# yashnaray/VQ-VAE-HMM-model

Measured on AMD Instinct MI355X. Metric: VAE_HMM train-step sequences/sec (K=3, T=200, D=5) at 1/2/4/8 MI355X, higher is better.
Workload: dtype f32; 1 GPU; cfg2: VAE_HMM train step (compute_loss+backward+Adam); global_batch=1024, per_gpu_batch=1024, seq_len=200, K=3, input_dim=5, hidden_dim=64, hidden_dim2=32, u_dim=4, trans_hidden=128, parallelism=single, hip_graph=False, step_form=fused (Adam in the backward's tail launch), eager

## Files before the change

### vq-vae-hmm-model_amd/csrc/strip.hip

```cpp
#include "vqhmm.h"

#include <stddef.h>
#include <stdlib.h>

#include "prof.h"
#include "strip_dev.h"

namespace vqhmm {

struct StripFwdArgs {
  int64_t R;
  int T, D, H2, K, P;
  const float* xp;
  const float *img_e1, *img_d1;
  const float *img_e2, *img_d2;
  const float *b_e1, *b_e2, *b_d1, *b_d2;
  const float *tWl, *tbl;
  const float *tWp, *tbp;
  float *h1e, *h2e, *logits, *q, *g1, *g2, *par;
  int64_t nstrip;
  int dbg;
};

namespace {

template <int NB2>
struct StripFwdLds {
  static constexpr int NW2 = 16 * NB2;
  float We2[3 * NW2 * ST_LDW];
  float Wd2[3 * 64 * ST_LDW];
  float Ee2[NW2 * 17 + 16];
  float Ed2[64 * 17 + 16];
  float Wf[2][3 * 64 * 8];
  float bf[2][64];
  float Xx[ST_XR * ST_XLD];
  float Xq[ST_XR * ST_XLD];
  float slot[8][18 * ST_LDW];
  unsigned long long hcnt[8];
};

template <int TH>
struct StripHeadW {
  static constexpr int LDW2 = TH + 4;
  float W2S[16 * LDW2];
  float W1S[TH * 8];
};
struct StripHeadLds {
  static constexpr int LDL = 20;
  float uS[ST_WIN * 8];
  float lgS[ST_WIN * LDL];
  float dlgS[ST_WIN * LDL];
  float aS[ST_WIN * 4];
  float wS[ST_WIN];
  double red[8][4];
  float q0w[8][4];
};

__device__ __forceinline__ void pk_weights(const float* Wf, int C, int lg4, int l16, float (&w)[4][4]) {
#pragma unroll
  for (int e = 0; e < 4; ++e) {
    const int k = 4 * lg4 + e;
    const bool in = k < 3 * C;
    const int tap = in ? k / C : 0, c = in ? k - tap * C : 0;
#pragma unroll
    for (int nb = 0; nb < 4; ++nb) {
      const float v = Wf[(tap * 64 + nb * 16 + l16) * 8 + c];
      w[nb][e] = in ? v : 0.f;
    }
  }
}

__device__ __forceinline__ void pk_block(const float (&w)[4][4], const float* Xw, int C, int lg4, int l16,
                                         f32x4 (&acc)[4]) {
  float b[4];
#pragma unroll
  for (int e = 0; e < 4; ++e) {
    const int k = 4 * lg4 + e;
    const bool in = k < 3 * C;
    const int tap = in ? k / C : 0, c = in ? k - tap * C : 0;
    const float v = Xw[(l16 + tap) * ST_XLD + c];
    b[e] = in ? v : 0.f;
  }
#pragma unroll
  for (int nb = 0; nb < 4; ++nb) {
    acc[nb] = f32x4{0.f, 0.f, 0.f, 0.f};
#pragma unroll
    for (int e = 0; e < 4; ++e) acc[nb] = mfma16x16x4(w[nb][e], b[e], acc[nb]);
  }
}

__device__ __forceinline__ void front_epi(f32x4 (&acc)[4], const f32x4 (&bias)[4], int64_t r0, int64_t R, int T,
                                          int lg4, int l16, int slo, int shi, float* out, float* xs,
                                          bool nostore, int only = -1, float* xlo = nullptr,
                                          float* xhi = nullptr) {
  const int64_t r = r0 + l16;
  const bool valid = row_valid(r, R, T);
  const bool st = l16 >= slo && l16 < shi && r < R && !nostore;
#pragma unroll
  for (int nb = 0; nb < 4; ++nb) {
    f32x4 y;
#pragma unroll
    for (int v = 0; v < 4; ++v) {
      const float yy = relu_f(acc[nb][v] * 1.0f + bias[nb][v]);
      y[v] = valid ? yy : 0.f;
    }
    acc[nb] = y;
    if (st) *reinterpret_cast<f32x4*>(out + r * 64 + nb * 16 + 4 * lg4) = y;
    if (only < 0 || l16 == only) *reinterpret_cast<f32x4*>(xs + l16 * ST_LDW + nb * 16 + 4 * lg4) = y;
    if (xlo && l16 == 0) *reinterpret_cast<f32x4*>(xlo + nb * 16 + 4 * lg4) = y;
    if (xhi && l16 == 15) *reinterpret_cast<f32x4*>(xhi + nb * 16 + 4 * lg4) = y;
  }
}

template <int NB>
struct TailConsts {
  f32x4 bias[NB], tw[NB], tb;
  __device__ __forceinline__ void load(const float* Es, int lg4, int l16) {
    constexpr int NW = 16 * NB;
#pragma unroll
    for (int nb = 0; nb < NB; ++nb) {
      const float4 b4 = *reinterpret_cast<const float4*>(Es + nb * 16 + 4 * lg4);
      const float4 t4 = *reinterpret_cast<const float4*>(Es + NW + l16 * NW + nb * 16 + 4 * lg4);
      bias[nb] = f32x4{b4.x, b4.y, b4.z, b4.w};
      tw[nb] = f32x4{t4.x, t4.y, t4.z, t4.w};
    }
    const float4 t4 = *reinterpret_cast<const float4*>(Es + 17 * NW + 4 * lg4);
    tb = f32x4{t4.x, t4.y, t4.z, t4.w};
  }
};

template <int NB, bool SM>
__device__ __forceinline__ void tail_epi(f32x4 (&acc)[NB], const TailConsts<NB>& k, int64_t r0, int64_t R, int T,
                                         int lg4, int l16, int slo, int shi, int N, float* out, int C2, float* t_out,
                                         float* q_out, float* xq, bool nostore) {
  const int64_t r = r0 + l16;
  const bool valid = row_valid(r, R, T);
  const bool st = l16 >= slo && l16 < shi && r < R && !nostore;
  const int ldn = ld4(N), ldt = ld4(C2);
#pragma unroll
  for (int nb = 0; nb < NB; ++nb) {
    f32x4 y;
#pragma unroll
    for (int v = 0; v < 4; ++v) {
      const float yy = relu_f(acc[nb][v] * 1.0f + k.bias[nb][v]);
      y[v] = valid ? yy : 0.f;
    }
    acc[nb] = y;
    const int n0 = nb * 16 + 4 * lg4;
    if (st && n0 < ldn) *reinterpret_cast<f32x4*>(out + r * ldn + n0) = y;
  }
  f32x4 z = k.tb;
#pragma unroll
  for (int nb = 0; nb < NB; ++nb)
#pragma unroll
    for (int v = 0; v < 4; ++v) z = mfma16x16x4(k.tw[nb][v], acc[nb][v], z);
  const int c0 = 4 * lg4;
#pragma unroll
  for (int v = 0; v < 4; ++v) z[v] = valid ? z[v] : 0.f;
  if (st && c0 < ldt) *reinterpret_cast<f32x4*>(t_out + r * ldt + c0) = z;
  if constexpr (SM) {
    float m = -__builtin_inff();
#pragma unroll
    for (int v = 0; v < 4; ++v)
      if (c0 + v < C2) m = fmaxf(m, z[v]);
    m = fmaxf(m, xor16(m));
    m = fmaxf(m, xor32(m));
    float e[4], s = 0.f;
#pragma unroll
    for (int v = 0; v < 4; ++v) {
      e[v] = (c0 + v < C2) ? __expf(z[v] - m) : 0.f;
      s += e[v];
    }
    s += xor16(s);
    s += xor32(s);
    f32x4 qv;
#pragma unroll
    for (int v = 0; v < 4; ++v) qv[v] = valid ? e[v] / s : 0.f;
    if (st && c0 < ldt) *reinterpret_cast<f32x4*>(q_out + r * ldt + c0) = qv;
    if (c0 == 0) {
      *reinterpret_cast<f32x4*>(xq + l16 * ST_XLD) = qv;
      *reinterpret_cast<f32x4*>(xq + l16 * ST_XLD + 4) = z;
    }
  }
}

template <int NW>
__device__ __forceinline__ const float* es_src(const float* bias, int N, const float* tW, const float* tb, int C2, int i,
                                               bool& ok) {
  const bool in_b = i < NW, in_w = !in_b && i < 17 * NW;
  const int j = in_w ? i - NW : 0, c2w = j / NW, n = j - c2w * NW, c2b = (!in_b && !in_w) ? i - 17 * NW : 0;
  ok = in_b ? i < N : in_w ? (c2w < C2 && n < N) : c2b < C2;
// ... 12 lines not shown
}
__device__ __forceinline__ float row4_max(float v) {
  v = fmaxf(v, dppf<0xB1>(v));
  v = fmaxf(v, dppf<0x4E>(v));
  return v;
}
__device__ __forceinline__ float row4_reduce_scatter(const float (&c)[4], int i) {
  const bool hi2 = i & 2, hi1 = i & 1;
  float h2[2];
#pragma unroll
  for (int k = 0; k < 2; ++k) {
    const float send = hi2 ? c[k] : c[2 + k];
    h2[k] = (hi2 ? c[2 + k] : c[k]) + dppf<0x4E>(send);
  }
  const float send = hi1 ? h2[0] : h2[1];
  return (hi1 ? h2[1] : h2[0]) + dppf<0xB1>(send);
}
}

template <int NB2, int PROF, int HTH>
__global__ __launch_bounds__(512) void strip_fwd_kernel(StripFwdArgs a, HeadArgs h) {
  using S = StripFwdLds<NB2>;
  constexpr int NW2 = S::NW2;
  extern __shared__ float4 smem4[];
  S& sh = *reinterpret_cast<S*>(smem4);
  const int tid = threadIdx.x, lane = tid & 63, wave = tid >> 6;
  const int lg4 = lane >> 4, l16 = lane & 15;
  const int64_t R = a.R;
  const int T = a.T, ldx = ld4(a.D);
  float* slot = sh.slot[wave];

  auto load_x = [&](int64_t s0) {
    const int row = tid >> 1, h = 4 * (tid & 1);
    int64_t r = s0 - 2 + row;
    r = r < 0 ? 0 : (r >= R ? R - 1 : r);
    return *reinterpret_cast<const float4*>(a.xp + r * ldx + (h < ldx ? h : 0));
  };
  auto store_x = [&](int64_t s0, float4 v) {
    if (tid < 2 * ST_XR) {
      const int row = tid >> 1, h = 4 * (tid & 1);
      const int64_t r = s0 - 2 + row;
      const bool ok = r >= 0 && r < R && h < ldx;
      *reinterpret_cast<float4*>(sh.Xx + row * ST_XLD + h) = ok ? v : make_float4(0.f, 0.f, 0.f, 0.f);
    }
  };

  constexpr int HKP = 4, HB = HTH > 0 ? HTH / 16 : 1, HLDW2 = HTH + 4, HNW = HTH > 0 ? 16 * HLDW2 + HTH * 8 : 1;
  constexpr int HNJ = (HNW + 511) / 512;
  const int prow = tid >> 2, si = tid & 3;
  float hwv[HNJ];
  if constexpr (HTH > 0) {
    const int KK = h.K * h.K;
#pragma unroll
    for (int j = 0; j < HNJ; ++j) {
      const int i = tid + 512 * j;
      float v = 0.f;
      if (i < 16 * HLDW2) {
        const int ij = i / HLDW2, hh = i - ij * HLDW2;
        v = (ij < KK && hh < HTH) ? h.W2[ij * HTH + hh] : 0.f;
      } else if (i < HNW) {
        const int k = i - 16 * HLDW2, hh = k >> 3, c = k & 7;
        v = c < h.U ? h.W1[hh * h.U + c] : (c == h.U ? h.b1[hh] : 0.f);
      }
      hwv[j] = v;
    }
    if (!h.norm && !h.cnt_in) {
      unsigned long long c = 0;
      for (int64_t b = tid; b < h.B; b += 512) {
        const int64_t L = h.lengths[b];
        c += (unsigned long long)(L <= 0 ? 0 : (L < T ? L : T));
      }
#pragma unroll
      for (int o = 32; o >= 1; o >>= 1) c += __shfl_xor(c, o);
      if (lane == 0) sh.hcnt[wave] = c;
    }
  }
  stamp<PROF>(0);
  if constexpr (PROF > 0) { if (threadIdx.x == 0 && blockIdx.x < 256) g_prof[blockIdx.x * 16 + 13] = __builtin_amdgcn_s_memtime(); }
  for (int j = wave; wave < 4 && j < 12; j += 4) {
    const int g = j * 64 + lane, img = g / 384, i = g - img * 384, row = i >> 1, h = 4 * (i & 1);
    dma16((img ? a.img_d1 : a.img_e1) + row * ST_LDF + h, &sh.Wf[0][0] + j * 256);
  }
  int64_t s = blockIdx.x;
  float4 px = load_x(s * ST_OWN - ST_HALO);
  constexpr int NE = NW2 * 17 + 16, ND = 64 * 17 + 16, NC = NE + ND + 128;
  constexpr int NCJ = (NC + 511) / 512;
  float cv[NCJ];
  bool cvok[NCJ];
#pragma unroll
  for (int j = 0; j < NCJ; ++j) {
    const int i = tid + 512 * j;
    bool oke, okd;
    const float* pe = es_src<NW2>(a.b_e2, a.H2, a.tWl, a.tbl, a.K, i < NE ? i : 0, oke);
    const float* pd = es_src<64>(a.b_d2, 64, a.tWp, a.tbp, a.P, (i >= NE && i < NE + ND) ? i - NE : 0, okd);
    const int ib = (i >= NE + ND && i < NC) ? i - NE - ND : 0;
    const bool inE = i < NE, inD = !inE && i < NE + ND, inB = !inE && !inD && i < NC;
    const bool ok = inE ? oke : inD ? okd : inB;
    const float* p = inE ? pe : inD ? pd : (ib < 64 ? a.b_e1 : a.b_d1) + (ib & 63);
    cv[j] = *(ok ? p : a.b_e1);
    cvok[j] = ok;
  }
#pragma unroll
  for (int j = 0; j < NCJ; ++j) cv[j] = cvok[j] ? cv[j] : 0.f;
  {
    constexpr int N1 = 3 * NW2 * ST_LDW / 4, N2 = 3 * 64 * ST_LDW / 4;
    constexpr int C1 = (N1 + 63) / 64, C2 = (N2 + 63) / 64;
    constexpr int NJ = (C1 + C2 + 7) / 8;
#pragma unroll
    for (int jj = 0; jj < NJ; ++jj) {
      const int c = min(wave + 8 * jj, C1 + C2 - 1);
      const bool first = c < C1;
      const int cc = first ? c : c - C1;
      const int i = cc * 64 + lane;
      if (i < (first ? N1 : N2)) dma16((first ? a.img_e2 : a.img_d2) + 4 * i, (first ? sh.We2 : sh.Wd2) + cc * 256);
    }
  }
  static_assert(offsetof(S, Ed2) == offsetof(S, Ee2) + NE * 4, "constant blocks must be contiguous");
#pragma unroll
  for (int j = 0; j < NCJ; ++j) {
    const int i = tid + 512 * j;
    if (i < NE + ND) sh.Ee2[i] = cv[j];
    else if (i < NC) sh.bf[0][i - NE - ND] = cv[j];
  }
  if (tid < 4 * ST_XLD) sh.Xq[(tid < 2 * ST_XLD ? 0 : (ST_XR - 4) * ST_XLD) + tid] = 0.f;
  store_x(s * ST_OWN - ST_HALO, px);
  lds_barrier();
  stamp<PROF>(1);
  float wE[4][4], wD[4][4];
  pk_weights(sh.Wf[0], a.D, lg4, l16, wE);
  pk_weights(sh.Wf[1], a.K, lg4, l16, wD);
  f32x4 bE[4], bD[4];
#pragma unroll
  for (int nb = 0; nb < 4; ++nb) {
    const float4 e4 = *reinterpret_cast<const float4*>(sh.bf[0] + nb * 16 + 4 * lg4);
    const float4 d4 = *reinterpret_cast<const float4*>(sh.bf[1] + nb * 16 + 4 * lg4);
    bE[nb] = f32x4{e4.x, e4.y, e4.z, e4.w};
    bD[nb] = f32x4{d4.x, d4.y, d4.z, d4.w};
  }
  TailConsts<NB2> kE;
  TailConsts<4> kD;
  if constexpr (HTH == 0) {
    kE.load(sh.Ee2, lg4, l16);
    kD.load(sh.Ed2, lg4, l16);
  }
  static_assert(HTH == 0 || (offsetof(S, Xx) == offsetof(S, bf) + 2 * 64 * 4 &&
                             sizeof(StripHeadW<HTH>) <= offsetof(S, Xx) - offsetof(S, Wf) &&
                             sizeof(StripHeadLds) <= sizeof(float) * 8 * 18 * ST_LDW),
                "the head's LDS fits the regions it reuses");
  float lp_i = 0.f, inv_n = 1.f, cpri = 0.f, cent = 0.f;
  const bool hgrad = h.need_grad != 0;
  if constexpr (HTH > 0) {
    unsigned long long cnt;
    if (h.norm) cnt = (unsigned long long)h.norm[0];
    else if (h.cnt_in) cnt = (unsigned long long)*h.cnt_in;
    else cnt = ((((((sh.hcnt[0] + sh.hcnt[1]) + sh.hcnt[2]) + sh.hcnt[3]) + sh.hcnt[4]) + sh.hcnt[5]) + sh.hcnt[6]) + sh.hcnt[7];
    inv_n = 1.0f / fmaxf((float)(cnt * (unsigned long long)h.D), 1.0f);
    const float Bn = loss_norm_batch(h.norm, h.B);
    cpri = -h.beta / Bn;
    cent = h.beta / Bn;
    float m = -__builtin_inff();
    for (int k = 0; k < h.K; ++k) m = fmaxf(m, h.log_prior[k]);
    float se = 0.f;
    for (int k = 0; k < h.K; ++k) se += __expf(h.log_prior[k] - m);
    if (si < h.K) lp_i = h.log_prior[si] - (m + __logf(se));
  }
  float s_rec = 0.f, s_ent = 0.f, s_tr = 0.f, s_init = 0.f, q0acc = 0.f, db2acc = 0.f;
  f32x4 gW2 = f32x4{0.f, 0.f, 0.f, 0.f}, gW1 = gW2;

  const int mlo = ST_HALO - 16 * wave, mhi = ST_HALO + ST_OWN - 16 * wave;
  const int slo = max(0, mlo), shi = min(16, mhi);
  const bool nost = a.dbg & 1;
  int it = 0;
  for (; s < a.nstrip; s += gridDim.x) {
    const int64_t s0 = s * ST_OWN - ST_HALO;
    const int64_t rb = s0 + 16 * wave;
    {
      const int64_t nx = s + gridDim.x;
      px = load_x((nx < a.nstrip ? nx : s) * ST_OWN - ST_HALO);
    }
    {
      f32x4 acc[4];
      pk_block(wE, sh.Xx + (16 * wave + 1) * ST_XLD, a.D, lg4, l16, acc);
      front_epi(acc, bE, rb, R, T, lg4, l16, slo, shi, a.h1e, slot + ST_LDW, nost, -1,
                wave > 0 ? sh.slot[wave - 1] + 17 * ST_LDW : nullptr, wave < 7 ? sh.slot[wave + 1] : nullptr);
      if (wave == 5 || wave == 6) {
        const bool lo = wave == 5;
        f32x4 acc2[4];
        pk_block(wE, sh.Xx + (lo ? 0 : 16 * 7 + 2) * ST_XLD, a.D, lg4, l16, acc2);
        front_epi(acc2, bE, lo ? s0 - 1 : s0 + 16 * 7 + 1, R, T, lg4, l16, 0, 0, a.h1e,
                  lo ? sh.slot[0] : sh.slot[7] + 2 * ST_LDW, true, lo ? 0 : 15);
      }
    }
    if (it == 0) asm volatile("s_waitcnt vmcnt(0)" ::: "memory");
    lds_barrier();
    {
      f32x4 acc[NB2][1];
#pragma unroll
      for (int nb = 0; nb < NB2; ++nb) acc[nb][0] = f32x4{0.f, 0.f, 0.f, 0.f};
      c2_mfma_tile<NB2, 1, 4, 3, ST_LDW, NW2>(sh.We2, slot, lg4, l16, acc, true);
      f32x4 y[NB2];
#pragma unroll
      for (int nb = 0; nb < NB2; ++nb) y[nb] = acc[nb][0];
      if constexpr (HTH > 0) kE.load(sh.Ee2, lg4, l16);
      tail_epi<NB2, true>(y, kE, rb, R, T, lg4, l16, slo, shi, a.H2, a.h2e, a.K, a.logits, a.q,
                          sh.Xq + (16 * wave + 2) * ST_XLD, nost);
    }
    lds_barrier();
    if (it == 0) stamp<PROF>(2);
    if constexpr (HTH > 0) {
      if (it == 0) {
        float* hw = &sh.Wf[0][0];
#pragma unroll
        for (int j = 0; j < HNJ; ++j)
          if (tid + 512 * j < HNW) hw[tid + 512 * j] = hwv[j];
      }
    }
    {
      f32x4 acc[4];
      pk_block(wD, sh.Xq + (16 * wave + 1) * ST_XLD, a.K, lg4, l16, acc);
      if constexpr (PROF > 0) {
        if (it == 0) {
          asm volatile("s_nop 0" : : "v"(acc[3][3]));
          stamp<PROF>(10);
        }
      }
      front_epi(acc, bD, rb, R, T, lg4, l16, slo, shi, a.g1, slot + ST_LDW, nost, -1,
                wave > 0 ? sh.slot[wave - 1] + 17 * ST_LDW : nullptr, wave < 7 ? sh.slot[wave + 1] : nullptr);
      if (it == 0) stamp<PROF>(11);
    }
    lds_barrier();
    if (it == 0) stamp<PROF>(4);
    {
      f32x4 acc[4][1];
#pragma unroll
      for (int nb = 0; nb < 4; ++nb) acc[nb][0] = f32x4{0.f, 0.f, 0.f, 0.f};
      c2_mfma_tile<4, 1, 4, 3, ST_LDW, 64>(sh.Wd2, slot, lg4, l16, acc, true);
      f32x4 y[4];
#pragma unroll
      for (int nb = 0; nb < 4; ++nb) y[nb] = acc[nb][0];
      if constexpr (PROF > 0) {
        if (it == 0) {
          asm volatile("s_nop 0" : : "v"(y[3][3]));
          stamp<PROF>(5);
        }
      }
      if constexpr (HTH > 0) kD.load(sh.Ed2, lg4, l16);
      tail_epi<4, false>(y, kD, rb, R, T, lg4, l16, slo, shi, 64, a.g2, a.P, a.par, nullptr, nullptr, nost);
    }
    if (it == 0) stamp<PROF>(6);
    {
      const int64_t nx = s + gridDim.x;
      store_x((nx < a.nstrip ? nx : s) * ST_OWN - ST_HALO, px);
    }
    if constexpr (HTH > 0) __syncthreads();
    else lds_barrier();
    if (it == 0) stamp<PROF>(3);
    if constexpr (HTH > 0) {
      StripHeadLds& hs = *reinterpret_cast<StripHeadLds*>(&sh.slot[0][0]);
      const StripHeadW<HTH>& hw = *reinterpret_cast<const StripHeadW<HTH>*>(&sh.Wf[0][0]);
      constexpr int LDL = StripHeadLds::LDL;
      const int K = h.K, U = h.U, D = h.D, KK = K * K;
      const int ldp = ld4(2 * D), ldxh = ld4(D), ldu = ld4(U);
      const int64_t r = s0 + ST_HALO + prow;
      const unsigned Tp = (unsigned)T + 2u;
      const unsigned rcl = (unsigned)(r < R ? r : R - 1);
      const int b = (int)(rcl / Tp);
      const int t = (int)(rcl - (unsigned)b * Tp) - 1;
      const bool valid = r < R && prow <= ST_OWN && t >= 0 && t < T;
      const bool own = prow < ST_OWN && r < R;
      const int64_t L = h.lengths[b];
      const bool m = valid && t < L;
      const float wgt = (valid && t >= 1 && t < L) ? 1.f : 0.f;
      const float* qrow = sh.Xq + (ST_HALO + prow + 2) * ST_XLD;
      float qv[HKP];
#pragma unroll
      for (int k = 0; k < HKP; ++k) qv[k] = (valid && k < K) ? qrow[k] : 0.f;
      const float qp = (valid && t >= 1 && si < K) ? qrow[si - ST_XLD] : 0.f;
      float qi = 0.f;
#pragma unroll
      for (int k = 0; k < HKP; ++k) qi = si == k ? qv[k] : qi;
      float mu[2], lv[2], xv[2];
#pragma unroll
      for (int k = 0; k < 2; ++k) {
        const int c = min(si + HKP * k, D - 1);
        mu[k] = h.par[(int64_t)rcl * ldp + c];
        lv[k] = h.par[(int64_t)rcl * ldp + D + c];
        xv[k] = h.x[(int64_t)rcl * ldxh + c];
      }
      const float uu = h.u[(int64_t)rcl * ldu + min(si, ldu - 1)];
#pragma unroll
      for (int c = si; c < 8; c += HKP) hs.uS[prow * 8 + c] = c < U ? (valid ? uu : 0.f) : (c == U ? 1.f : 0.f);
      for (int i = tid; i < ST_WIN * LDL; i += 512)
        if (i % LDL >= KK) hs.dlgS[i] = 0.f;
      lds_barrier();
      {
        f32x4 lg;
#pragma unroll
        for (int v = 0; v < 4; ++v) {
          const int ij = 4 * lg4 + v;
          lg[v] = ij < KK ? h.b2[ij] : 0.f;
        }
        const float ub = hs.uS[(wave * 16 + l16) * 8 + lg4];
#pragma unroll 2
        for (int hb = 0; hb < HB; ++hb) {
          const float w1a = lg4 < U ? hw.W1S[(hb * 16 + l16) * 8 + lg4] : 0.f;
          f32x4 bb;
#pragma unroll
          for (int v = 0; v < 4; ++v) bb[v] = hw.W1S[(hb * 16 + 4 * lg4 + v) * 8 + U];
          const f32x4 w2v = *reinterpret_cast<const f32x4*>(&hw.W2S[l16 * HLDW2 + hb * 16 + 4 * lg4]);
          const f32x4 hc = mfma16x16x4(w1a, ub, bb);
#pragma unroll
          for (int v = 0; v < 4; ++v) lg = mfma16x16x4(w2v[v], relu_f(hc[v]), lg);
        }
        *reinterpret_cast<f32x4*>(&hs.lgS[(wave * 16 + l16) * LDL + 4 * lg4]) = lg;
      }
      lds_barrier();
      float rsj = 0.f;
      {
        float la[HKP];
        float A_i = 0.f;
        const float* lr = &hs.lgS[prow * LDL + (si < K ? si : 0) * K];
        float mx = -__builtin_inff();
#pragma unroll
        for (int j = 0; j < HKP; ++j) {
          la[j] = j < K ? lr[j] : 0.f;
          if (j < K) mx = fmaxf(mx, la[j]);
        }
        float se = 0.f;
#pragma unroll
        for (int j = 0; j < HKP; ++j)
          if (j < K) se += __expf(la[j] - mx);
        const float ls = mx + __logf(se);
#pragma unroll
        for (int j = 0; j < HKP; ++j)
          if (j < K) la[j] -= ls;
#pragma unroll
        for (int j = 0; j < HKP; ++j)
          if (j < K) A_i = fmaf(qv[j], la[j], A_i);
        if (si >= K) A_i = 0.f;
        float c[HKP];
#pragma unroll
        for (int j = 0; j < HKP; ++j) c[j] = (j < K && si < K) ? qp * la[j] : 0.f;
        rsj = row4_reduce_scatter(c, si);
        if (own && si < K) s_tr = fmaf(wgt * qp, A_i, s_tr);
        hs.aS[prow * HKP + si] = A_i;
        if (si == 0) hs.wS[prow] = wgt;
        if (hgrad && si < K) {
          float qs = 0.f;
#pragma unroll
          for (int j = 0; j < HKP; ++j)
            if (j < K) qs += qv[j];
          const float g = own ? cpri * wgt * qp : 0.f;
          const float rs = g * qs;
          float* dl = &hs.dlgS[prow * LDL + si * K];
#pragma unroll
          for (int j = 0; j < HKP; ++j)
// ... 246 lines not shown
    lds_barrier();
    f32x4 d1[4];
    {
      f32x4 acc[4][1];
#pragma unroll
      for (int nb = 0; nb < 4; ++nb) acc[nb][0] = f32x4{0.f, 0.f, 0.f, 0.f};
      c2_mfma_tile<4, 1, 4, 3, ST_LDW, 64>(sh.Wd2, slot, lg4, l16, acc, true);
#pragma unroll
      for (int nb = 0; nb < 4; ++nb) d1[nb] = acc[nb][0];
      mask_epi(d1, m1, 1.0f, rb, R, T, lg4, l16, slo, shi, a.dg1, nullptr, 0);
    }
    lds_barrier();
#pragma unroll
    for (int nb = 0; nb < 4; ++nb) *reinterpret_cast<f32x4*>(D1 + (16 * wave + 1 + l16) * ST_LDW + nb * 16 + 4 * lg4) = d1[nb];
    float4 m2[4];
    load_mask(a.h1e, rb, R, lg4, l16, m2);
    lds_barrier();
    if (it == 0) stamp<PROF>(2);
    {
      f32x4 acc1[1][1] = {{f32x4{0.f, 0.f, 0.f, 0.f}}};
      c2_mfma_tile<1, 1, 4, 3, ST_LDW, 16>(sh.Wc1, D1 + 16 * wave * ST_LDW, lg4, l16, acc1, true);
      const float zb1[1][4] = {}, tw1[1][4] = {};
      const float4 aux1[1][1] = {};
      const float fsc = f.scale ? *f.scale : 1.0f;
      conv2_epilogue<1, 1, 3>(f, rb, 0, lg4, l16, acc1, aux1, zb1, tw1, f32x4{0.f, 0.f, 0.f, 0.f}, fsc, false, slo,
                              shi, sh.Dh2 + (16 * wave + 1) * SB_LDE, SB_LDE);
    }
    lds_barrier();
    if (it == 0) stamp<PROF>(3);
    {
      f32x4 acc[4][1];
#pragma unroll
      for (int nb = 0; nb < 4; ++nb) acc[nb][0] = f32x4{0.f, 0.f, 0.f, 0.f};
      c2_mfma_tile<4, 1, 2, 3, SB_LDE, 64>(sh.We2, sh.Dh2 + 16 * wave * SB_LDE, lg4, l16, acc, true);
      f32x4 y[4];
#pragma unroll
      for (int nb = 0; nb < 4; ++nb) y[nb] = acc[nb][0];
      mask_epi(y, m2, 1.0f, rb, R, T, lg4, l16, slo, shi, a.dh1, nullptr, 0);
    }
    ++it;
  }
  if constexpr (PROF > 0) {
    __syncthreads();
    stamp<PROF>(7);
    if (threadIdx.x == 0 && blockIdx.x < 256) g_prof[blockIdx.x * 16 + 8] = (unsigned long long)it;
  }
}

bool strip_bwd_supported(const ConvArgs& pd, const ConvArgs& d2, const ConvArgs& f, const ConvArgs& e2) {
  return pd.R > 0 && pd.R < (1ll << 31) && pd.ks == 1 && pd.act == 2 && pd.Wimg && pd.aux && pd.out && pd.N == 64 &&
         pd.Kc >= 1 && pd.Kc <= 16 && !pd.src_cf && !pd.bias &&
         d2.src == pd.out && d2.ks == 3 && d2.act == 2 && d2.Wimg && d2.aux && d2.out && d2.Kc == 64 && d2.N == 64 &&
         !d2.bias && !d2.scale &&
         f.src == d2.out && f.act == 3 && f.ks == 3 && f.Wimg && f.Kc == 64 && f.N >= 1 && f.N <= 4 && f.lb_dh &&
         f.lb_C > 16 && f.lb_C <= 32 && ld4(f.lb_C) == 32 && !f.bias && !f.out_cf &&
         e2.src == f.lb_dh && e2.ks == 3 && e2.act == 2 && e2.Wimg && e2.aux && e2.out && e2.Kc == f.lb_C &&
         e2.N == 64 && !e2.bias && !e2.scale && !e2.tW && !e2.out_cf;
}

int launch_strip_bwd(const ConvArgs& pd, const ConvArgs& d2, const ConvArgs& f, const ConvArgs& e2, hipStream_t s) {
  if (!strip_bwd_supported(pd, d2, f, e2)) return VQHMM_EUNSUPPORTED;
  StripBwdArgs a{};
  a.R = pd.R; a.T = pd.T; a.ldp = ld4(pd.Kc);
  a.dpar = pd.src; a.g2 = pd.aux; a.g1 = d2.aux; a.h1e = e2.aux;
  a.img_pd = pd.Wimg; a.img_d2 = d2.Wimg; a.img_c1 = f.Wimg; a.img_e2 = e2.Wimg;
  a.gscale = pd.scale;
  a.dg2 = pd.out; a.dg1 = d2.out; a.dh1 = e2.out;
  a.nstrip = cdiv(pd.R, ST_OWN);
  const unsigned grid = (unsigned)(a.nstrip < 256 ? a.nstrip : 256);
  if (prof_on()) strip_bwd_kernel<1><<<grid, 512, sizeof(StripBwdLds), s>>>(a, f);
  else strip_bwd_kernel<0><<<grid, 512, sizeof(StripBwdLds), s>>>(a, f);
  VQHMM_LAUNCH_CHECK();
  return VQHMM_OK;
}

static StripFwdArgs strip_fwd_args(const ConvArgs& e1, const ConvArgs& e2, const ConvArgs& d1, const ConvArgs& d2) {
  StripFwdArgs a{};
  a.R = e1.R; a.T = e1.T; a.D = e1.Kc; a.H2 = e2.N; a.K = e2.C2; a.P = d2.C2;
  a.xp = e1.src;
  a.img_e1 = e1.Wimg; a.img_d1 = d1.Wimg; a.img_e2 = e2.Wimg; a.img_d2 = d2.Wimg;
  a.b_e1 = e1.bias; a.b_e2 = e2.bias; a.b_d1 = d1.bias; a.b_d2 = d2.bias;
  a.tWl = e2.tW; a.tbl = e2.tb; a.tWp = d2.tW; a.tbp = d2.tb;
  a.h1e = e1.out; a.h2e = e2.out; a.logits = e2.t_out; a.q = e2.q_out; a.g1 = d1.out; a.g2 = d2.out; a.par = d2.t_out;
  a.nstrip = cdiv(e1.R, ST_OWN);
  static const int dbg = [] {
    const char* e = VQHMM_PROF_ENV("VQHMM_STRIP_DBG");
    return e ? atoi(e) : 0;
  }();
  a.dbg = dbg;
  return a;
}

bool strip_fwd_supported(const ConvArgs& e1, const ConvArgs& e2, const ConvArgs& d1, const ConvArgs& d2) {
  auto relu3 = [](const ConvArgs& a) { return a.ks == 3 && a.act == 1 && !a.src_cf && a.Wimg && a.out && !a.out_cf; };
  return relu3(e1) && relu3(e2) && relu3(d1) && relu3(d2) && e1.R > 0 && e1.R < (1ll << 31) &&
         e1.Kc >= 1 && 3 * e1.Kc <= 16 && e1.N == 64 &&
         e2.src == e1.out && e2.Kc == 64 && e2.N >= 1 && e2.N <= 32 &&
         e2.C2 >= 1 && e2.C2 <= 4 && e2.t_out && e2.q_out && !e2.q_cf && !e2.reg_out && !e2.t_cf0 &&
         d1.src == e2.q_out && d1.Kc == e2.C2 && 3 * d1.Kc <= 16 && d1.N == 64 &&
         d2.src == d1.out && d2.Kc == 64 && d2.N == 64 && d2.C2 >= 1 && d2.C2 <= 16 && d2.t_out && !d2.t_cf0 &&
         !d2.q_out && !d2.q_cf && !d2.reg_out;
}

int strip_prof_copy(uint64_t* out, int64_t n) { return prof_copy(out, n); }

bool strip_head_supported(const HeadArgs& h) {
  return h.K >= 1 && h.K <= 4 && h.U >= 1 && h.U <= 4 && (h.TH == 64 || h.TH == 128) && h.D >= 1 && h.D <= 8 &&
         h.R < (1ll << 31);
}

int strip_fwd_grid(int64_t R) {
  const int64_t n = cdiv(R, ST_OWN);
  return (int)(n < 256 ? (n > 0 ? n : 1) : 256);
}

int launch_strip_fwd(const ConvArgs& e1, const ConvArgs& e2, const ConvArgs& d1, const ConvArgs& d2, const HeadArgs* h,
                     hipStream_t s) {
  if (!strip_fwd_supported(e1, e2, d1, d2)) return VQHMM_EUNSUPPORTED;
  if (h && (!strip_head_supported(*h) || h->K != e2.C2 || h->R != e1.R || h->D != e1.Kc)) return VQHMM_EUNSUPPORTED;
  const StripFwdArgs a = strip_fwd_args(e1, e2, d1, d2);
  const unsigned grid = (unsigned)strip_fwd_grid(e1.R);
  const HeadArgs hv = h ? *h : HeadArgs{};
  const int hth = h ? h->TH : 0;
#define VQHMM_SF(NB2, P, HT) strip_fwd_kernel<NB2, P, HT><<<grid, 512, sizeof(StripFwdLds<NB2>), s>>>(a, hv)
#define VQHMM_SF_H(NB2, P) \
  if (hth == 128) VQHMM_SF(NB2, P, 128); else if (hth == 64) VQHMM_SF(NB2, P, 64); else VQHMM_SF(NB2, P, 0);
  const bool prof = prof_on() != 0;
  if (c2_nb(e2.N) == 1) {
    if (prof) { VQHMM_SF_H(1, 1) } else { VQHMM_SF_H(1, 0) }
  } else {
    if (prof) { VQHMM_SF_H(2, 1) } else { VQHMM_SF_H(2, 0) }
  }
#undef VQHMM_SF_H
#undef VQHMM_SF
  VQHMM_LAUNCH_CHECK();
  return VQHMM_OK;
}

}
```

### vq-vae-hmm-model_amd/csrc/strip_bwdw.hip

```cpp
#include "vqhmm.h"

#include <stddef.h>

#include "prof.h"
#include "strip_dev.h"

namespace vqhmm {

__device__ float g_bwdw_one = 1.0f;

namespace {
constexpr int SW_LDD = 24;
constexpr int SW_LDQ = 8;
constexpr int SW_LO = 3;
constexpr int SW_OWN = 120;
static_assert(SW_OWN % 4 == 0 && SW_LO + SW_OWN - 1 <= ST_WIN - 4, "dh1 is exact on window rows 3 .. ST_WIN - 4");

struct StripWLds {
  float RW[3 * 64 * ST_LDW];
  float RS[8 * 18 * ST_LDW];
  float RG[ST_WIN * ST_LDW];
  float RD[(ST_WIN + 2) * SB_LDE];
  float RC[4 * 256];
  float RE[ST_WIN * SW_LDQ];
// ... 65 lines not shown
    ar[j % NS] = fa(qa, j);
#pragma unroll
    for (int t = 0; t < NT; ++t) br[j % NS][t] = fb(qb, j, t);
  };
  auto load = [&](int j) __attribute__((always_inline)) { load_at(j, pa, pb); };
  auto next = [&]() __attribute__((always_inline)) {
    pa += ga;
    pb += gb;
    hide(pa);
    hide(pb);
  };
  hide(pa);
  hide(pb);
  auto mma = [&](int j) __attribute__((always_inline)) {
    const float av = (SEL == SEL_A && !ok) ? 0.f : ar[j % NS];
    bacc += av;
#pragma unroll
    for (int t = 0; t < NT; ++t) acc[t] = mfma16x16x4(av, (SEL == SEL_B && !ok) ? 0.f : br[j % NS][t], acc[t]);
  };
  if constexpr (NT == 1) {
    if (nstep < 4) {
#pragma unroll
      for (int j = 0; j < 3; ++j)
        if (j < nstep) load(j);
#pragma unroll
      for (int j = 0; j < 3; ++j)
        if (j < nstep) mma(j);
      return;
    }
#pragma unroll
    for (int j = 0; j < 4; ++j) {
      load(j);
      asm volatile("" ::: "memory");
    }
    next();
    int k = 0;
    for (; k + 8 <= nstep; k += 4) {
#pragma unroll
      for (int j = 0; j < 4; ++j) {
        __builtin_amdgcn_sched_barrier(0);
        mma(j);
        __builtin_amdgcn_sched_barrier(0);
        load(j);
      }
      next();
    }
    const int rem = nstep - k - 4;
#pragma unroll
    for (int j = 0; j < 4; ++j) {
      __builtin_amdgcn_sched_barrier(0);
      mma(j);
      __builtin_amdgcn_sched_barrier(0);
      if (j < 3) load_at(j, j < rem ? pa : pa - ga, j < rem ? pb : pb - gb);
    }
#pragma unroll
    for (int j = 0; j < 3; ++j) {
      __builtin_amdgcn_sched_barrier(0);
      if (j < rem) mma(j);
    }
    return;
  }
  load(0);
  int k = 0;
  for (; k + 5 <= nstep; k += 4) {
#pragma unroll
    for (int j = 0; j < 4; ++j) {
      if (j == 3) next();
      load((j + 1) & 3);
      __builtin_amdgcn_sched_barrier(0);
      mma(j);
      __builtin_amdgcn_sched_barrier(0);
    }
  }
  const int rem = nstep - k;
#pragma unroll
  for (int j = 0; j < 4; ++j) {
    if (j < 3 && j + 1 < rem) load(j + 1);
    __builtin_amdgcn_sched_barrier(0);
    if (j < rem) mma(j);
    __builtin_amdgcn_sched_barrier(0);
  }
}

__device__ __forceinline__ void dma16_uncounted(const float* src, int off, float* dst) {
  const unsigned d = __builtin_amdgcn_readfirstlane((unsigned)(size_t)(__attribute__((address_space(3))) float*)dst);
  unsigned keep;
  asm volatile("s_nop 4\n\ts_mov_b32 %0, m0\n\ts_mov_b32 m0, %2\n\ts_nop 0\n\t"
               "global_load_lds_dwordx4 %1, %3\n\ts_mov_b32 m0, %0"
               : "=&s"(keep)
               : "v"(off), "s"(d), "s"(src)
               : "memory");
}

__device__ __forceinline__ float col_sum4(float v) {
  v += xor16(v);
  v += xor32(v);
  return v;
}
__device__ __forceinline__ void dec1_epi(f32x4 acc, float sc, int64_t r, int64_t R, int T, int lg4, int l16, float lsc,
                                         const f32x4 (&qdl)[3], const f32x4 (&h4)[2], const float* TWs, float* xs_dh,
                                         float* xs_dl) {
  const bool valid = row_valid(r, R, T);
  f32x4 y;
#pragma unroll
  for (int v = 0; v < 4; ++v) {
    const float yy = acc[v] * sc + 0.f;
    y[v] = valid ? yy : 0.f;
  }
  float yk[4];
#pragma unroll
  for (int k = 0; k < 4; ++k) yk[k] = __shfl(y[k], l16);
  if (r >= 0 && r < R) {
    float dq[4], sdot = 0.f;
#pragma unroll
    for (int k = 0; k < 4; ++k) {
      dq[k] = yk[k] + lsc * qdl[1][k];
      sdot = fmaf(qdl[0][k], dq[k], sdot);
    }
    float dl[4];
#pragma unroll
    for (int k = 0; k < 4; ++k) dl[k] = qdl[0][k] * (dq[k] - sdot) + lsc * qdl[2][k];
    if (lg4 == 0) *reinterpret_cast<f32x4*>(xs_dl + l16 * SW_LDQ) = f32x4{dl[0], dl[1], dl[2], dl[3]};
#pragma unroll
    for (int j = 0; j < 2; ++j) {
      const int c0 = 8 * lg4 + 4 * j;
      f32x4 o;
#pragma unroll
      for (int v = 0; v < 4; ++v) {
        float sacc = 0.f;
#pragma unroll
        for (int k = 0; k < 4; ++k) sacc = fmaf(TWs[k * 32 + c0 + v], dl[k], sacc);
        o[v] = h4[j][v] > 0.f ? sacc : 0.f;
      }
      *reinterpret_cast<f32x4*>(xs_dh + l16 * SB_LDE + c0) = o;
    }
  } else {
#pragma unroll
    for (int j = 0; j < 2; ++j) *reinterpret_cast<f32x4*>(xs_dh + l16 * SB_LDE + 8 * lg4 + 4 * j) = f32x4{0.f, 0.f, 0.f, 0.f};
    if (lg4 == 0) *reinterpret_cast<f32x4*>(xs_dl + l16 * SW_LDQ) = f32x4{0.f, 0.f, 0.f, 0.f};
  }
}
}

template <int PROF>
__global__ __launch_bounds__(512) void strip_bwdw_kernel(SWArgs a, ConvArgs f) {
  extern __shared__ float4 smem4[];
  StripWLds& sh = *reinterpret_cast<StripWLds*>(smem4);
  const int tid = threadIdx.x, lane = tid & 63, wave = tid >> 6;
  const int lg4 = lane >> 4, l16 = lane & 15;
  const int64_t R = a.R;
  const int T = a.T, own = a.own, nstep = own / 4;
  constexpr int lo = SW_LO;
  float* slot = sh.RS + wave * 18 * ST_LDW;
  if (a.step_inc && blockIdx.x == 0 && tid == 0) *a.step_inc = (*a.step_inc & 0xffffffffll) + 1;

  stamp<PROF>(0);
  if constexpr (PROF > 0) { if (tid == 0 && blockIdx.x < 256) g_prof[blockIdx.x * 16 + 13] = __builtin_amdgcn_s_memtime(); }
  const int K = a.K, D = a.D;
  float twv = 0.f;
  if (tid < 128) {
    const int k = tid >> 5, c = tid & 31;
    twv = (k < K && c < a.H2) ? f.lb_W[k * a.H2 + c] : 0.f;
  }
  {
    constexpr int NC = 3 * 4 * ST_LDW / 4;
    static_assert(NC <= 4 * 64 && sizeof(StripWLds::RC) == 4 * 1024, "one whole-chunk DMA per wave");
    const int c = min(wave, 3);
    const int i = min(c * 64 + lane, NC - 1);
    dma16(a.img_c1 + ((i / 72) * 16 * ST_LDW + (i % 72) * 4), sh.RC + c * 256);
  }
  if (tid < 128) sh.TW[tid] = twv;
  auto dma_d2 = [&]() __attribute__((always_inline)) {
    constexpr int N1 = 3 * 64 * ST_LDW / 4, C1 = N1 / 64;
    static_assert(N1 % 64 == 0 && C1 <= 56, "7 whole chunks per wave");
#pragma unroll
// ... 432 lines not shown
```

### vq-vae-hmm-model_amd/csrc/strip_dev.h

```cpp
#pragma once
#include "conv2_dev.h"

namespace vqhmm {

namespace {
constexpr int ST_WIN = 128;
constexpr int ST_HALO = 2;
constexpr int ST_OWN = ST_WIN - 2 * ST_HALO;
constexpr int ST_XR = ST_WIN + 4;
constexpr int ST_XLD = 8;
constexpr int ST_LDW = 72;
constexpr int ST_LDF = 24;
constexpr int SB_LDE = 40;

__device__ __forceinline__ bool row_valid(int64_t r, int64_t R, int T) {
  if (r < 0 || r >= R) return false;
  const unsigned Tp = (unsigned)T + 2u, m = (unsigned)r % Tp;
  return m >= 1u && m <= (unsigned)T;
}

__device__ __forceinline__ void lds_barrier_dma() { asm volatile("s_waitcnt lgkmcnt(0)\n\ts_barrier" ::: "memory"); }

__device__ __forceinline__ void dma16(const float* src, float* dst) {
  __builtin_amdgcn_global_load_lds(reinterpret_cast<const uint32_t*>(src), (__attribute__((address_space(3))) void*)dst,
                                   16, 0, 0);
}

__device__ __forceinline__ void mask_epi(f32x4 (&acc)[4], const float4 (&aux)[4], float sc, int64_t r0, int64_t R,
                                         int T, int lg4, int l16, int slo, int shi, float* out, float* xs, int xld,
                                         int only = -1, float* xlo = nullptr, float* xhi = nullptr) {
  const int64_t r = r0 + l16;
  const bool valid = row_valid(r, R, T);
  const bool st = out && l16 >= slo && l16 < shi && r < R;
#pragma unroll
  for (int nb = 0; nb < 4; ++nb) {
    const float av[4] = {aux[nb].x, aux[nb].y, aux[nb].z, aux[nb].w};
    f32x4 y;
#pragma unroll
    for (int v = 0; v < 4; ++v) {
      float yy = acc[nb][v] * sc + 0.f;
      yy = av[v] > 0.f ? yy : 0.f;
      y[v] = valid ? yy : 0.f;
    }
    acc[nb] = y;
    if (st) *reinterpret_cast<f32x4*>(out + r * 64 + nb * 16 + 4 * lg4) = y;
    if (xs && (only < 0 || l16 == only)) *reinterpret_cast<f32x4*>(xs + l16 * xld + nb * 16 + 4 * lg4) = y;
    if (xlo && l16 == 0) *reinterpret_cast<f32x4*>(xlo + nb * 16 + 4 * lg4) = y;
    if (xhi && l16 == 15) *reinterpret_cast<f32x4*>(xhi + nb * 16 + 4 * lg4) = y;
  }
}

__device__ __forceinline__ void load_mask(const float* m, int64_t r0, int64_t R, int lg4, int l16, float4 (&aux)[4]) {
  int64_t r = r0 + l16;
  r = r < 0 ? 0 : (r >= R ? R - 1 : r);
#pragma unroll
  for (int nb = 0; nb < 4; ++nb) aux[nb] = *reinterpret_cast<const float4*>(m + r * 64 + nb * 16 + 4 * lg4);
}
}

}
```

Baseline: 2.662 million sequences/s.

## Widen strip halo to drop extra edge conv blocks in strip forward

Changes the strip forward kernel's owned window from 124 rows with a 2-row halo to 122 rows starting at row 3. This lets the extra per-strip edge-row conv work done by waves 5 and 6 be removed, since the edge values are now recomputed inside the window. It also precomputes the conv gather offsets once, moves the weight-image DMA after the x store using an uncounted LDS DMA helper, and moves the next-strip x store earlier in the loop. The trade-off is slightly more strips and halo overlap, plus more reliance on hand-written asm DMA ordering.

```diff
diff --git a/vq-vae-hmm-model_amd/csrc/strip.hip b/vq-vae-hmm-model_amd/csrc/strip.hip
--- a/vq-vae-hmm-model_amd/csrc/strip.hip
+++ b/vq-vae-hmm-model_amd/csrc/strip.hip
@@ -23,6 +23,10 @@
 };
 
 namespace {
+
+constexpr int SF_LO = 3;
+constexpr int SF_OWN = 122;
+static_assert(SF_LO >= 3 && SF_LO + SF_OWN - 1 <= ST_WIN - 4, "g2 / par are exact on window rows 3 .. ST_WIN - 4");
 
 template <int NB2>
 struct StripFwdLds {
@@ -70,17 +74,30 @@
   }
 }
 
-__device__ __forceinline__ void pk_block(const float (&w)[4][4], const float* Xw, int C, int lg4, int l16,
-                                         f32x4 (&acc)[4]) {
+struct PkGather {
+  int off[4];
+  unsigned in;
+  __device__ __forceinline__ void set(int C, int lg4, int l16) {
+    in = 0;
+#pragma unroll
+    for (int e = 0; e < 4; ++e) {
+      const int k = 4 * lg4 + e;
+      const bool ok = k < 3 * C;
+      const int tap = ok ? k / C : 0, c = ok ? k - tap * C : 0;
+      off[e] = (l16 + tap) * ST_XLD + c;
+      asm volatile("" : "+v"(off[e]));
+      in |= ok ? 1u << e : 0u;
+    }
+  }
+};
+
+__device__ __forceinline__ void pk_block(const float (&w)[4][4], const float* Xw, const PkGather& g, f32x4 (&acc)[4]) {
   float b[4];
 #pragma unroll
-  for (int e = 0; e < 4; ++e) {
-    const int k = 4 * lg4 + e;
-    const bool in = k < 3 * C;
-    const int tap = in ? k / C : 0, c = in ? k - tap * C : 0;
-    const float v = Xw[(l16 + tap) * ST_XLD + c];
-    b[e] = in ? v : 0.f;
-  }
+  for (int e = 0; e < 4; ++e) b[e] = Xw[g.off[e]];
+  __builtin_amdgcn_sched_barrier(0);
+#pragma unroll
+  for (int e = 0; e < 4; ++e) b[e] = (g.in >> e & 1u) ? b[e] : 0.f;
 #pragma unroll
   for (int nb = 0; nb < 4; ++nb) {
     acc[nb] = f32x4{0.f, 0.f, 0.f, 0.f};
@@ -91,8 +108,7 @@
 
 __device__ __forceinline__ void front_epi(f32x4 (&acc)[4], const f32x4 (&bias)[4], int64_t r0, int64_t R, int T,
                                           int lg4, int l16, int slo, int shi, float* out, float* xs,
-                                          bool nostore, int only = -1, float* xlo = nullptr,
-                                          float* xhi = nullptr) {
+                                          bool nostore, float* xlo = nullptr, float* xhi = nullptr) {
   const int64_t r = r0 + l16;
   const bool valid = row_valid(r, R, T);
   const bool st = l16 >= slo && l16 < shi && r < R && !nostore;
@@ -106,7 +122,7 @@
     }
     acc[nb] = y;
     if (st) *reinterpret_cast<f32x4*>(out + r * 64 + nb * 16 + 4 * lg4) = y;
-    if (only < 0 || l16 == only) *reinterpret_cast<f32x4*>(xs + l16 * ST_LDW + nb * 16 + 4 * lg4) = y;
+    *reinterpret_cast<f32x4*>(xs + l16 * ST_LDW + nb * 16 + 4 * lg4) = y;
     if (xlo && l16 == 0) *reinterpret_cast<f32x4*>(xlo + nb * 16 + 4 * lg4) = y;
     if (xhi && l16 == 15) *reinterpret_cast<f32x4*>(xhi + nb * 16 + 4 * lg4) = y;
   }
@@ -285,7 +301,7 @@
     dma16((img ? a.img_d1 : a.img_e1) + row * ST_LDF + h, &sh.Wf[0][0] + j * 256);
   }
   int64_t s = blockIdx.x;
-  float4 px = load_x(s * ST_OWN - ST_HALO);
+  float4 px = load_x(s * SF_OWN - SF_LO);
   constexpr int NE = NW2 * 17 + 16, ND = 64 * 17 + 16, NC = NE + ND + 128;
   constexpr int NCJ = (NC + 511) / 512;
   float cv[NCJ];
@@ -305,19 +321,6 @@
   }
 #pragma unroll
   for (int j = 0; j < NCJ; ++j) cv[j] = cvok[j] ? cv[j] : 0.f;
-  {
-    constexpr int N1 = 3 * NW2 * ST_LDW / 4, N2 = 3 * 64 * ST_LDW / 4;
-    constexpr int C1 = (N1 + 63) / 64, C2 = (N2 + 63) / 64;
-    constexpr int NJ = (C1 + C2 + 7) / 8;
-#pragma unroll
-    for (int jj = 0; jj < NJ; ++jj) {
-      const int c = min(wave + 8 * jj, C1 + C2 - 1);
-      const bool first = c < C1;
-      const int cc = first ? c : c - C1;
-      const int i = cc * 64 + lane;
-      if (i < (first ? N1 : N2)) dma16((first ? a.img_e2 : a.img_d2) + 4 * i, (first ? sh.We2 : sh.Wd2) + cc * 256);
-    }
-  }
   static_assert(offsetof(S, Ed2) == offsetof(S, Ee2) + NE * 4, "constant blocks must be contiguous");
 #pragma unroll
   for (int j = 0; j < NCJ; ++j) {
@@ -326,12 +329,29 @@
     else if (i < NC) sh.bf[0][i - NE - ND] = cv[j];
   }
   if (tid < 4 * ST_XLD) sh.Xq[(tid < 2 * ST_XLD ? 0 : (ST_XR - 4) * ST_XLD) + tid] = 0.f;
-  store_x(s * ST_OWN - ST_HALO, px);
+  store_x(s * SF_OWN - SF_LO, px);
+  {
+    constexpr int N1 = 3 * NW2 * ST_LDW / 4, N2 = 3 * 64 * ST_LDW / 4;
+    constexpr int C1 = (N1 + 63) / 64, C2 = (N2 + 63) / 64;
+    static_assert(N1 >= 64 && N2 >= 64, "a chunk is a whole KB inside its image");
+    constexpr int NJ = (C1 + C2 + 7) / 8;
+    const int wv = __builtin_amdgcn_readfirstlane(wave);
+#pragma unroll
+    for (int jj = 0; jj < NJ; ++jj) {
+      const int c = min(wv + 8 * jj, C1 + C2 - 1);
+      const bool first = c < C1;
+      const int i0 = first ? min(c * 64, N1 - 64) : min((c - C1) * 64, N2 - 64);
+      dma16_uncounted((first ? a.img_e2 : a.img_d2) + 4 * i0, 16 * lane, (first ? sh.We2 : sh.Wd2) + 4 * i0);
+    }
+  }
   lds_barrier();
   stamp<PROF>(1);
   float wE[4][4], wD[4][4];
   pk_weights(sh.Wf[0], a.D, lg4, l16, wE);
   pk_weights(sh.Wf[1], a.K, lg4, l16, wD);
+  PkGather gE, gD;
+  gE.set(a.D, lg4, l16);
+  gD.set(a.K, lg4, l16);
   f32x4 bE[4], bD[4];
 #pragma unroll
   for (int nb = 0; nb < 4; ++nb) {
@@ -370,29 +390,22 @@
   float s_rec = 0.f, s_ent = 0.f, s_tr = 0.f, s_init = 0.f, q0acc = 0.f, db2acc = 0.f;
   f32x4 gW2 = f32x4{0.f, 0.f, 0.f, 0.f}, gW1 = gW2;
 
-  const int mlo = ST_HALO - 16 * wave, mhi = ST_HALO + ST_OWN - 16 * wave;
+  const int mlo = SF_LO - 16 * wave, mhi = SF_LO + SF_OWN - 16 * wave;
   const int slo = max(0, mlo), shi = min(16, mhi);
   const bool nost = a.dbg & 1;
   int it = 0;
   for (; s < a.nstrip; s += gridDim.x) {
-    const int64_t s0 = s * ST_OWN - ST_HALO;
+    const int64_t s0 = s * SF_OWN - SF_LO;
     const int64_t rb = s0 + 16 * wave;
     {
       const int64_t nx = s + gridDim.x;
-      px = load_x((nx < a.nstrip ? nx : s) * ST_OWN - ST_HALO);
+      px = load_x((nx < a.nstrip ? nx : s) * SF_OWN - SF_LO);
     }
     {
       f32x4 acc[4];
-      pk_block(wE, sh.Xx + (16 * wave + 1) * ST_XLD, a.D, lg4, l16, acc);
-      front_epi(acc, bE, rb, R, T, lg4, l16, slo, shi, a.h1e, slot + ST_LDW, nost, -1,
+      pk_block(wE, sh.Xx + (16 * wave + 1) * ST_XLD, gE, acc);
+      front_epi(acc, bE, rb, R, T, lg4, l16, slo, shi, a.h1e, slot + ST_LDW, nost,
                 wave > 0 ? sh.slot[wave - 1] + 17 * ST_LDW : nullptr, wave < 7 ? sh.slot[wave + 1] : nullptr);
-      if (wave == 5 || wave == 6) {
-        const bool lo = wave == 5;
-        f32x4 acc2[4];
-        pk_block(wE, sh.Xx + (lo ? 0 : 16 * 7 + 2) * ST_XLD, a.D, lg4, l16, acc2);
-        front_epi(acc2, bE, lo ? s0 - 1 : s0 + 16 * 7 + 1, R, T, lg4, l16, 0, 0, a.h1e,
-                  lo ? sh.slot[0] : sh.slot[7] + 2 * ST_LDW, true, lo ? 0 : 15);
-      }
     }
     if (it == 0) asm volatile("s_waitcnt vmcnt(0)" ::: "memory");
     lds_barrier();
@@ -420,14 +433,14 @@
     }
     {
       f32x4 acc[4];
-      pk_block(wD, sh.Xq + (16 * wave + 1) * ST_XLD, a.K, lg4, l16, acc);
+      pk_block(wD, sh.Xq + (16 * wave + 1) * ST_XLD, gD, acc);
       if constexpr (PROF > 0) {
         if (it == 0) {
           asm volatile("s_nop 0" : : "v"(acc[3][3]));
           stamp<PROF>(10);
         }
       }
-      front_epi(acc, bD, rb, R, T, lg4, l16, slo, shi, a.g1, slot + ST_LDW, nost, -1,
+      front_epi(acc, bD, rb, R, T, lg4, l16, slo, shi, a.g1, slot + ST_LDW, nost,
                 wave > 0 ? sh.slot[wave - 1] + 17 * ST_LDW : nullptr, wave < 7 ? sh.slot[wave + 1] : nullptr);
       if (it == 0) stamp<PROF>(11);
     }
@@ -447,14 +460,14 @@
           stamp<PROF>(5);
         }
       }
+      {
+        const int64_t nx = s + gridDim.x;
+        store_x((nx < a.nstrip ? nx : s) * SF_OWN - SF_LO, px);
+      }
       if constexpr (HTH > 0) kD.load(sh.Ed2, lg4, l16);
       tail_epi<4, false>(y, kD, rb, R, T, lg4, l16, slo, shi, 64, a.g2, a.P, a.par, nullptr, nullptr, nost);
     }
     if (it == 0) stamp<PROF>(6);
-    {
-      const int64_t nx = s + gridDim.x;
-      store_x((nx < a.nstrip ? nx : s) * ST_OWN - ST_HALO, px);
-    }
     if constexpr (HTH > 0) __syncthreads();
     else lds_barrier();
     if (it == 0) stamp<PROF>(3);
@@ -464,17 +477,17 @@
       constexpr int LDL = StripHeadLds::LDL;
       const int K = h.K, U = h.U, D = h.D, KK = K * K;
       const int ldp = ld4(2 * D), ldxh = ld4(D), ldu = ld4(U);
-      const int64_t r = s0 + ST_HALO + prow;
+      const int64_t r = s0 + SF_LO + prow;
       const unsigned Tp = (unsigned)T + 2u;
       const unsigned rcl = (unsigned)(r < R ? r : R - 1);
       const int b = (int)(rcl / Tp);
       const int t = (int)(rcl - (unsigned)b * Tp) - 1;
-      const bool valid = r < R && prow <= ST_OWN && t >= 0 && t < T;
-      const bool own = prow < ST_OWN && r < R;
+      const bool valid = r < R && prow <= SF_OWN && t >= 0 && t < T;
+      const bool own = prow < SF_OWN && r < R;
       const int64_t L = h.lengths[b];
       const bool m = valid && t < L;
       const float wgt = (valid && t >= 1 && t < L) ? 1.f : 0.f;
-      const float* qrow = sh.Xq + (ST_HALO + prow + 2) * ST_XLD;
+      const float* qrow = sh.Xq + min(SF_LO + prow + 2, ST_XR - 1) * ST_XLD;
       float qv[HKP];
 #pragma unroll
       for (int k = 0; k < HKP; ++k) qv[k] = (valid && k < K) ? qrow[k] : 0.f;
@@ -887,7 +900,7 @@
   a.b_e1 = e1.bias; a.b_e2 = e2.bias; a.b_d1 = d1.bias; a.b_d2 = d2.bias;
   a.tWl = e2.tW; a.tbl = e2.tb; a.tWp = d2.tW; a.tbp = d2.tb;
   a.h1e = e1.out; a.h2e = e2.out; a.logits = e2.t_out; a.q = e2.q_out; a.g1 = d1.out; a.g2 = d2.out; a.par = d2.t_out;
-  a.nstrip = cdiv(e1.R, ST_OWN);
+  a.nstrip = cdiv(e1.R, SF_OWN);
   static const int dbg = [] {
     const char* e = VQHMM_PROF_ENV("VQHMM_STRIP_DBG");
     return e ? atoi(e) : 0;
@@ -915,7 +928,7 @@
 }
 
 int strip_fwd_grid(int64_t R) {
-  const int64_t n = cdiv(R, ST_OWN);
+  const int64_t n = cdiv(R, SF_OWN);
   return (int)(n < 256 ? (n > 0 ? n : 1) : 256);
 }
 
diff --git a/vq-vae-hmm-model_amd/csrc/strip_bwdw.hip b/vq-vae-hmm-model_amd/csrc/strip_bwdw.hip
--- a/vq-vae-hmm-model_amd/csrc/strip_bwdw.hip
+++ b/vq-vae-hmm-model_amd/csrc/strip_bwdw.hip
@@ -171,15 +171,6 @@
   }
 }
 
-__device__ __forceinline__ void dma16_uncounted(const float* src, int off, float* dst) {
-  const unsigned d = __builtin_amdgcn_readfirstlane((unsigned)(size_t)(__attribute__((address_space(3))) float*)dst);
-  unsigned keep;
-  asm volatile("s_nop 4\n\ts_mov_b32 %0, m0\n\ts_mov_b32 m0, %2\n\ts_nop 0\n\t"
-               "global_load_lds_dwordx4 %1, %3\n\ts_mov_b32 m0, %0"
-               : "=&s"(keep)
-               : "v"(off), "s"(d), "s"(src)
-               : "memory");
-}
 
 __device__ __forceinline__ float col_sum4(float v) {
   v += xor16(v);
diff --git a/vq-vae-hmm-model_amd/csrc/strip_dev.h b/vq-vae-hmm-model_amd/csrc/strip_dev.h
--- a/vq-vae-hmm-model_amd/csrc/strip_dev.h
+++ b/vq-vae-hmm-model_amd/csrc/strip_dev.h
@@ -24,6 +24,16 @@
 __device__ __forceinline__ void dma16(const float* src, float* dst) {
   __builtin_amdgcn_global_load_lds(reinterpret_cast<const uint32_t*>(src), (__attribute__((address_space(3))) void*)dst,
                                    16, 0, 0);
+}
+
+__device__ __forceinline__ void dma16_uncounted(const float* src, int off, float* dst) {
+  const unsigned d = __builtin_amdgcn_readfirstlane((unsigned)(size_t)(__attribute__((address_space(3))) float*)dst);
+  unsigned keep;
+  asm volatile("s_nop 4\n\ts_mov_b32 %0, m0\n\ts_mov_b32 m0, %2\n\ts_nop 0\n\t"
+               "global_load_lds_dwordx4 %1, %3\n\ts_mov_b32 m0, %0"
+               : "=&s"(keep)
+               : "v"(off), "s"(d), "s"(src)
+               : "memory");
 }
 
 __device__ __forceinline__ void mask_epi(f32x4 (&acc)[4], const float4 (&aux)[4], float sc, int64_t r0, int64_t R,
```

After: 2.708 million sequences/s (median of 6 runs). 1.02x the previous value.
